# rdspring1/lightning-thunder

Measured on AMD Instinct MI355X. Metric: tokens/sec/GPU Llama-2-7B pretrain (LitGPT) + speedup vs eager at 1/2/4/8 MI355X, higher is better.
Workload: dtype bf16; 1 GPU; model=Llama-2-7b-hf, global_batch=1, micro_batch=1, seq_len=4096, parallelism=single, mode=thunder, optimizer=AdamW

## Files before the change

### lightning_thunder_amd/ops/csrc/gemm4.hip

```cpp
#include "common.h"

using namespace lta;

namespace {

typedef __bf16 bf16x8 __attribute__((ext_vector_type(8)));
typedef short s16x4 __attribute__((ext_vector_type(4)));
typedef float f32x4 __attribute__((ext_vector_type(4)));
typedef int i32x4 __attribute__((ext_vector_type(4)));
typedef __attribute__((address_space(3))) void lds_void;
typedef __attribute__((address_space(3))) s16x4 lds_s16x4;

constexpr int BM = 256, BN = 256, BK = 64, NTHR = 256;
constexpr int OP_BYTES = BM * BK * 2;
constexpr int STAGE = 2 * OP_BYTES;

enum Act : int { kNone = 0, kGeluTanh = 1, kGeluErf = 2, kSilu = 3, kRelu = 4 };

template <int ACT>
__device__ __forceinline__ float act_fn(float x) {
  if constexpr (ACT == kGeluTanh) {
    const float u = 0.7978845608028654f * (x + 0.044715f * x * x * x);
    return 0.5f * x * (1.f + tanhf(u));
  } else if constexpr (ACT == kGeluErf) {
    return 0.5f * x * (1.f + erff(x * 0.7071067811865476f));
  } else if constexpr (ACT == kSilu) {
    return x / (1.f + __expf(-x));
  } else if constexpr (ACT == kRelu) {
    return x > 0.f ? x : 0.f;
  } else {
    return x;
  }
}

__device__ __forceinline__ int xcd_tile(int orig, int nwg) {
  const int xcd = orig & 7, q = nwg >> 3, r = nwg & 7;
  return (xcd < r ? xcd * (q + 1) : r * (q + 1) + (xcd - r) * q) + (orig >> 3);
}

__device__ __forceinline__ int tr_swz(int k) { return ((k & 3) | (((k >> 3) & 1) << 2)) << 1; }

__device__ __forceinline__ i32x4 make_rsrc(const void* base, int bytes) {
  const uint64_t a = (uint64_t)(uintptr_t)base;
  return i32x4{(int)(uint32_t)a, (int)((uint32_t)(a >> 32) & 0xffffu), bytes, 0x00020000};
}

template <bool MN, bool DUAL = false, bool KEDGE = false>
struct Stager {
  i32x4 rsrc, rsrc2;
  const char* kbase;
  int kred, ldb2;
  int voff[8];
  int istride, kstride;
  __device__ __forceinline__ void init(const __hip_bfloat16* X, int ld, int r0, int K, int wave, int lane,
                                       const __hip_bfloat16* X2 = nullptr, int valid = BM) {
    if constexpr (DUAL) {
      rsrc = make_rsrc(X + (int64_t)r0 * ld, (BM / 2 - 1) * ld * 2 + K * 2);
      rsrc2 = make_rsrc(X2 + (int64_t)r0 * ld, (BM / 2 - 1) * ld * 2 + K * 2);
      const int r = lane >> 3, c = (lane & 7) ^ r;
      voff[0] = ((wave * 8 + r) * ld + c * 8) * 2;
      istride = 32 * ld * 2;
      kstride = BK * 2;
    } else if constexpr (!MN) {
      const __hip_bfloat16* base = X + (int64_t)r0 * ld;
      rsrc = make_rsrc(base, (BM - 1) * ld * 2 + K * 2);
      const int r = lane >> 3, c = (lane & 7) ^ r;
#pragma unroll
      for (int i = 0; i < 8; ++i) voff[i] = (min(32 * i + wave * 8 + r, valid - 1) * ld + c * 8) * 2;
      istride = 0;
      kstride = BK * 2;
    } else {
      const __hip_bfloat16* base = X + r0;
      rsrc = make_rsrc(base, (K - 1) * ld * 2 + BM * 2);
      const int half = lane >> 5, slot = lane & 31;
      const int kr = 2 * wave + half;
      const int c0 = slot ^ tr_swz(kr), cmax = (valid >> 3) - 1;
      if constexpr (KEDGE) {
#pragma unroll
        for (int i = 0; i < 8; ++i) voff[i] = ((8 * i + kr) * ld + min((i & 1) ? c0 ^ 8 : c0, cmax) * 8) * 2;
        kbase = reinterpret_cast<const char*>(base);
        kred = K;
        ldb2 = ld * 2;
      } else {
        voff[0] = (kr * ld + min(c0, cmax) * 8) * 2;
        voff[1] = (kr * ld + min(c0 ^ 8, cmax) * 8) * 2;
      }
      istride = 8 * ld * 2;
      kstride = BK * ld * 2;
    }
  }
  __device__ __forceinline__ void issue(int i, int kt, char* img, int wave) const {
    const uint32_t dst = (uint32_t)(uintptr_t)(__attribute__((address_space(3))) char*)(img + (i * 4 + wave) * 1024);
    if constexpr (KEDGE) {
      const int rows = max(0, min(BK, kred - kt * BK));
      const uint64_t a = (uint64_t)(uintptr_t)(kbase + (int64_t)kt * BK * ldb2);
      const i32x4 rk = i32x4{__builtin_amdgcn_readfirstlane((int)(uint32_t)a),
                             __builtin_amdgcn_readfirstlane((int)((uint32_t)(a >> 32) & 0xffffu)),
                             __builtin_amdgcn_readfirstlane(rows * ldb2), 0x00020000};
      asm volatile("s_mov_b32 m0, %0\n\ts_nop 0\n\tbuffer_load_dwordx4 %1, %2, 0 offen lds"
                   :
                   : "s"(dst), "v"(voff[i]), "s"(rk)
                   : "memory", "m0");
      return;
    }
    const bool second = DUAL && ((i >> 1) & 1);
    const int vo = DUAL ? voff[0] : (MN ? voff[i & 1] : voff[i]);
    const int so = DUAL ? (2 * (i >> 2) + (i & 1)) * istride + kt * kstride
                        : (MN ? i * istride + kt * kstride : kt * kstride);
    asm volatile("s_mov_b32 m0, %0\n\ts_nop 0\n\tbuffer_load_dwordx4 %1, %2, %3 offen lds"
                 :
                 : "s"(dst), "v"(vo), "s"(second ? rsrc2 : rsrc), "s"(so)
                 : "memory", "m0");
  }
};

template <bool MN>
__device__ __forceinline__ bf16x8 read_frag(const char* img, int rc, int kk, int fr, int fq) {
  if constexpr (!MN) {
    const int row = rc + fr;
    return *reinterpret_cast<const bf16x8*>(img + row * 128 + (((kk * 4 + fq) ^ (fr & 7)) << 4));
  } else {
    const int q = fr >> 2, p = fr & 3;
    const int k = kk * 32 + fq * 8 + q;
    const int c = (rc >> 3) + (p >> 1);
    const char* a0 = img + k * 512 + ((c ^ tr_swz(k)) << 4) + 8 * (p & 1);
    const char* a1 = img + (k + 4) * 512 + ((c ^ tr_swz(k + 4)) << 4) + 8 * (p & 1);
    const s16x4 lo = __builtin_amdgcn_ds_read_tr16_b64_v4i16((lds_s16x4*)(__attribute__((address_space(3))) char*)a0);
    const s16x4 hi = __builtin_amdgcn_ds_read_tr16_b64_v4i16((lds_s16x4*)(__attribute__((address_space(3))) char*)a1);
    union {
      struct {
        s16x4 a, b;
      } s;
      bf16x8 f;
    } u;
    u.s.a = lo;
    u.s.b = hi;
    return u.f;
  }
}

#define LTA_FENCE() __builtin_amdgcn_sched_barrier(0)

__device__ __forceinline__ void mfma16(f32x4& acc, const bf16x8& a, const bf16x8& b) {
  asm volatile("v_mfma_f32_16x16x32_bf16 %0, %1, %2, %0" : "+a"(acc) : "v"(a), "v"(b));
}

__device__ __forceinline__ float sigmoid_f(float x) { return 1.f / (1.f + __expf(-x)); }

__device__ __forceinline__ float bf16_round(float x) { return __bfloat162float(__float2bfloat16(x)); }

typedef float f32x2_t __attribute__((ext_vector_type(2)));
typedef __bf16 bf16x2_t __attribute__((ext_vector_type(2)));
__device__ __forceinline__ uint32_t pack_bf16x2(float lo, float hi) {
  return __builtin_bit_cast(uint32_t, __builtin_convertvector(f32x2_t{lo, hi}, bf16x2_t));
}

__device__ __forceinline__ uint4 swap_pair(uint32_t x0, uint32_t x1, uint32_t y0, uint32_t y1) {
  const auto s0 = __builtin_amdgcn_permlane16_swap(x0, y0, false, false);
  const auto s1 = __builtin_amdgcn_permlane16_swap(x1, y1, false, false);
  return make_uint4(s0[0], s1[0], s0[1], s1[1]);
}

struct EpiArgs {
  const __hip_bfloat16* B2;
  __hip_bfloat16* C2;
  __hip_bfloat16* C3;
  const __hip_bfloat16* R2;
  const float* cos_;
  const float* sin_;
  int T, nh, ng;
  const int* offs;
  int G;
  int64_t bstride, cstride;
  int tile_base, tile_count, ksplit;
  float* partial;
};

__device__ __forceinline__ void tile_coords(int wg, int nTm, int nTn, int& tm, int& tn) {
  constexpr int G = 8;
  const int per_group = G * nTn;
  const int group = wg / per_group;
  const int first_m = group * G;
  const int gm = min(nTm - first_m, G);
  const int in_group = wg % per_group;
  tm = first_m + in_group % gm;
  tn = in_group / gm;
}

template <int ACT, bool BIAS, bool RES, bool AT, bool BT, int VAR, int EPI = 0, int GRP = 0, int TAIL = 0>
__global__ __launch_bounds__(NTHR, 1) void gemm4_bf16_kernel(const __hip_bfloat16* __restrict__ A,
                                                            const __hip_bfloat16* __restrict__ B,
                                                            __hip_bfloat16* __restrict__ C,
                                                            const __hip_bfloat16* __restrict__ bias,
                                                            const __hip_bfloat16* __restrict__ R, int M, int N, int K,
                                                            int lda, int ldb, int ldc, int ldr, float alpha,
                                                            EpiArgs ep = {}) {
  const __hip_bfloat16* const B2 = ep.B2;
  __hip_bfloat16* const C2 = ep.C2;
  __hip_bfloat16* const C3 = ep.C3;
  const __hip_bfloat16* const R2 = ep.R2;
  static_assert(EPI != 1 || (!AT && !BT && !BIAS && !RES && ACT == 0), "gate-up: forward layout, no other epilogue");
  static_assert(EPI != 3 || (!AT && !BT && !BIAS && !RES && ACT == 0), "qkv rope: forward layout, no other epilogue");
  static_assert(EPI != 2 || (!AT && BT && !BIAS && !RES && ACT == 0), "swiglu backward: dgrad layout only");
  static_assert(GRP == 0 || (EPI == 0 && !BIAS && !RES && ACT == 0), "grouped: plain products");
  static_assert(GRP != 1 || !AT, "grouped rows: A row-major");
  static_assert(GRP != 2 || (AT && BT), "grouped reduction: A and B stored [rows][.]");
  constexpr bool SW = true;
  __shared__ __attribute__((aligned(1024))) char smem[2 * STAGE];

  const int tid = threadIdx.x, lane = tid & 63;
  const int wave = __builtin_amdgcn_readfirstlane(tid >> 6);
  const int wm = wave >> 1, wn = wave & 1;
  const int fr = lane & 15, fq = lane >> 4;

  const int nTm = (M + BM - 1) / BM, nTn = (N + BN - 1) / BN, nwg = nTm * nTn;
  const __hip_bfloat16* Ag = A;
  const __hip_bfloat16* Bg = B;
  __hip_bfloat16* Cg = C;
  int Mlim = M, Kr = K, m0, n0;
  [[maybe_unused]] int wg_lin = 0, kpart = 0;
  if constexpr (GRP == 0) {
    int wg;
    if constexpr (TAIL == 2) {
      const int t = __builtin_amdgcn_readfirstlane((int)blockIdx.x / ep.ksplit);
      kpart = __builtin_amdgcn_readfirstlane((int)blockIdx.x - t * ep.ksplit);
      wg = ep.tile_base + t;
    }
    else if constexpr (TAIL == 1)
      wg = ep.tile_base + xcd_tile((int)blockIdx.x, ep.tile_count);
    else
      wg = xcd_tile((int)blockIdx.x, nwg);
    wg_lin = wg;
    int tm, tn;
    tile_coords(wg, nTm, nTn, tm, tn);
    m0 = tm * BM;
    n0 = tn * BN;
    if constexpr (TAIL == 2) {
      const int P = K / (2 * BK), q = __builtin_amdgcn_readfirstlane(P / ep.ksplit), r = P - q * ep.ksplit;
      const int k0 = (kpart * q + min(kpart, r)) * (2 * BK);
      Kr = (q + (kpart < r ? 1 : 0)) * (2 * BK);
      Ag = A + (AT ? (int64_t)k0 * lda : (int64_t)k0);
      Bg = B + (BT ? (int64_t)k0 * ldb : (int64_t)k0);
    }
  } else if constexpr (GRP == 1) {
    const int bid = (int)blockIdx.x, tn = bid % nTn;
    int slot = bid / nTn, g = 0, start = 0, end = 0;
    bool found = false;
    for (; g < ep.G; ++g) {
      end = ep.offs[g];
      const int tiles = (end - start + BM - 1) / BM;
      if (slot < tiles) {
        found = true;
        break;
      }
      slot -= tiles;
      start = end;
    }
    if (!found) return;
    m0 = start + slot * BM;
    n0 = tn * BN;
    Mlim = end;
    Bg = B + (int64_t)g * ep.bstride;
  } else {
    const int g = (int)blockIdx.x / nwg, t = (int)blockIdx.x % nwg;
    const int start = g ? ep.offs[g - 1] : 0, end = ep.offs[g];
    m0 = (t / nTn) * BM;
    n0 = (t % nTn) * BN;
    Ag = A + (int64_t)start * lda;
    Bg = B + (int64_t)start * ldb;
    Cg = C + (int64_t)g * ep.cstride;
// ... 510 lines not shown
  ep.tile_base = 0;
  ep.tile_count = nwg - tail;
  hipLaunchKernelGGL((gemm4_bf16_kernel<kNone, false, false, AT, BT, 1, 0, 0, 1>), dim3(nwg - tail), dim3(NTHR), 0, s,
                     (const __hip_bfloat16*)A, (const __hip_bfloat16*)B, (__hip_bfloat16*)C, nullptr, nullptr, M, N, K,
                     lda, ldb, ldc, 0, alpha, ep);
  ep.tile_base = nwg - tail;
  ep.tile_count = tail;
  ep.ksplit = 2;
  ep.partial = (float*)ws;
  hipLaunchKernelGGL((gemm4_bf16_kernel<kNone, false, false, AT, BT, 1, 0, 0, 2>), dim3(2 * tail), dim3(NTHR), 0, s,
                     (const __hip_bfloat16*)A, (const __hip_bfloat16*)B, (__hip_bfloat16*)C, nullptr, nullptr, M, N, K,
                     lda, ldb, ldc, 0, 1.f, ep);
  hipLaunchKernelGGL(gemm4_tail_fixup, dim3((unsigned)((int64_t)tail * (BM * BN / 8) / 256)), dim3(256), 0, s,
                     (const float*)ws, (__hip_bfloat16*)C, 2, nwg - tail, tail, M, N, ldc, alpha);
  return (int)hipGetLastError();
}

template <bool AT, bool BT>
int launch4_splitk(const void* A, const void* B, void* C, const void* bias, int M, int N, int K, int lda, int ldb,
                   int ldc, float alpha, int ksplit, void* ws, int64_t ws_bytes, hipStream_t s) {
  const int nwg = ((M + BM - 1) / BM) * ((N + BN - 1) / BN);
  if (ksplit < 2 || ksplit > 64 || K % (2 * BK) || K / (2 * BK) < ksplit || !ws ||
      ws_bytes < (int64_t)ksplit * nwg * BM * BN * 4)
    return -2;
  EpiArgs ep{};
  ep.tile_base = 0;
  ep.tile_count = nwg;
  ep.ksplit = ksplit;
  ep.partial = (float*)ws;
  hipLaunchKernelGGL((gemm4_bf16_kernel<kNone, false, false, AT, BT, 1, 0, 0, 2>), dim3(ksplit * nwg), dim3(NTHR), 0,
                     s, (const __hip_bfloat16*)A, (const __hip_bfloat16*)B, (__hip_bfloat16*)C, nullptr, nullptr, M, N,
                     K, lda, ldb, ldc, 0, 1.f, ep);
  hipLaunchKernelGGL(gemm4_tail_fixup, dim3((unsigned)((int64_t)nwg * (BM * BN / 8) / 256)), dim3(256), 0, s,
                     (const float*)ws, (__hip_bfloat16*)C, ksplit, 0, nwg, M, N, ldc, alpha,
                     (const __hip_bfloat16*)bias);
  return (int)hipGetLastError();
}

template <int ACT, bool AT, bool BT, int VAR>
int launch4(const void* A, const void* B, void* C, const void* bias, const void* R, int M, int N, int K, int lda,
            int ldb, int ldc, int ldr, float alpha, hipStream_t s) {
  dim3 grid(((M + BM - 1) / BM) * ((N + BN - 1) / BN)), block(NTHR);
#define LTA_G4(BI, RE)                                                                                            \
  hipLaunchKernelGGL((gemm4_bf16_kernel<ACT, BI, RE, AT, BT, VAR>), grid, block, 0, s, (const __hip_bfloat16*)A,  \
                     (const __hip_bfloat16*)B, (__hip_bfloat16*)C, (const __hip_bfloat16*)bias,                  \
                     (const __hip_bfloat16*)R, M, N, K, lda, ldb, ldc, ldr, alpha)
  if (bias && R) { LTA_G4(true, true); }
  else if (bias) { LTA_G4(true, false); }
  else if (R) { LTA_G4(false, true); }
  else { LTA_G4(false, false); }
#undef LTA_G4
  return (int)hipGetLastError();
}

template <int VAR>
int dispatch_layout(const void* A, const void* B, void* C, const void* bias, const void* R, int M, int N, int K,
                    int lda, int ldb, int ldc, int ldr, float alpha, int act, int at, int bt, hipStream_t s) {
  if (!at && !bt) {
    switch (act) {
      case kNone: return launch4<kNone, false, false, VAR>(A, B, C, bias, R, M, N, K, lda, ldb, ldc, ldr, alpha, s);
      case kGeluTanh: return launch4<kGeluTanh, false, false, VAR>(A, B, C, bias, R, M, N, K, lda, ldb, ldc, ldr, alpha, s);
      case kGeluErf: return launch4<kGeluErf, false, false, VAR>(A, B, C, bias, R, M, N, K, lda, ldb, ldc, ldr, alpha, s);
      case kSilu: return launch4<kSilu, false, false, VAR>(A, B, C, bias, R, M, N, K, lda, ldb, ldc, ldr, alpha, s);
      case kRelu: return launch4<kRelu, false, false, VAR>(A, B, C, bias, R, M, N, K, lda, ldb, ldc, ldr, alpha, s);
      default: return -1;
    }
  }
  if (act != kNone || bias) return -1;
  if (!at && bt) return launch4<kNone, false, true, VAR>(A, B, C, nullptr, R, M, N, K, lda, ldb, ldc, ldr, alpha, s);
  if (at && !bt) return launch4<kNone, true, false, VAR>(A, B, C, nullptr, R, M, N, K, lda, ldb, ldc, ldr, alpha, s);
  return launch4<kNone, true, true, VAR>(A, B, C, nullptr, R, M, N, K, lda, ldb, ldc, ldr, alpha, s);
}

}

LTA_EXPORT int lta_gemm4_bf16(const void* A, const void* B, void* C, const void* bias, const void* R, int M, int N,
                              int K, int lda, int ldb, int ldc, int ldr, float alpha, int act, int at, int bt,
                              int variant, hipStream_t s) {
  if (N % 8 || K % (2 * BK) || M <= 0 || N <= 0 || K <= 0) return -2;
  if (at && M % 8) return -2;
  const int64_t ea = at ? (int64_t)K * lda : (int64_t)M * lda, eb = bt ? (int64_t)K * ldb : (int64_t)N * ldb;
  if (ea * 2 >= (1ll << 31) || eb * 2 >= (1ll << 31)) return -2;
  if (variant != 1) return -1;
  return dispatch_layout<1>(A, B, C, bias, R, M, N, K, lda, ldb, ldc, ldr, alpha, act, at, bt, s);
}

LTA_EXPORT int lta_gemm4_bf16_ws(const void* A, const void* B, void* C, const void* bias, const void* R, int M, int N,
                                 int K, int lda, int ldb, int ldc, int ldr, float alpha, int act, int at, int bt,
                                 int variant, void* ws, int64_t ws_bytes, hipStream_t s) {
  if (ws && variant == 1 && act == kNone && !bias && !R && N % 8 == 0 && M > 0 && N > 0 && K > 0 && !(at && M % 8)) {
    const int64_t ea = at ? (int64_t)K * lda : (int64_t)M * lda, eb = bt ? (int64_t)K * ldb : (int64_t)N * ldb;
    if (ea * 2 < (1ll << 31) && eb * 2 < (1ll << 31)) {
      int rc = -1;
      if (!at && !bt) rc = launch4_tail<false, false>(A, B, C, M, N, K, lda, ldb, ldc, alpha, ws, ws_bytes, s);
      else if (!at && bt) rc = launch4_tail<false, true>(A, B, C, M, N, K, lda, ldb, ldc, alpha, ws, ws_bytes, s);
      else if (at && !bt) rc = launch4_tail<true, false>(A, B, C, M, N, K, lda, ldb, ldc, alpha, ws, ws_bytes, s);
      else rc = launch4_tail<true, true>(A, B, C, M, N, K, lda, ldb, ldc, alpha, ws, ws_bytes, s);
      if (rc != -1) return rc;
    }
  }
  return lta_gemm4_bf16(A, B, C, bias, R, M, N, K, lda, ldb, ldc, ldr, alpha, act, at, bt, variant, s);
}

LTA_EXPORT int lta_gemm4_bf16_splitk(const void* A, const void* B, void* C, const void* bias, int M, int N, int K,
                                     int lda, int ldb, int ldc, float alpha, int at, int bt, int ksplit, void* ws,
                                     int64_t ws_bytes, hipStream_t s) {
  if (N % 8 || M <= 0 || N <= 0 || K <= 0 || (at && M % 8) || (bias && (at || bt))) return -2;
  const int64_t ea = at ? (int64_t)K * lda : (int64_t)M * lda, eb = bt ? (int64_t)K * ldb : (int64_t)N * ldb;
  if (ea * 2 >= (1ll << 31) || eb * 2 >= (1ll << 31)) return -2;
  if (!at && !bt) return launch4_splitk<false, false>(A, B, C, bias, M, N, K, lda, ldb, ldc, alpha, ksplit, ws, ws_bytes, s);
  if (!at && bt) return launch4_splitk<false, true>(A, B, C, bias, M, N, K, lda, ldb, ldc, alpha, ksplit, ws, ws_bytes, s);
  if (at && !bt) return launch4_splitk<true, false>(A, B, C, bias, M, N, K, lda, ldb, ldc, alpha, ksplit, ws, ws_bytes, s);
  return launch4_splitk<true, true>(A, B, C, bias, M, N, K, lda, ldb, ldc, alpha, ksplit, ws, ws_bytes, s);
}

LTA_EXPORT int lta_gemm4_grouped(int mode, const void* A, const void* B, void* C, const void* offs, int G, int M, int N,
                                 int K, int lda, int ldb, int ldc, int64_t bstride, int64_t cstride, int bt,
                                 hipStream_t s) {
  if (G <= 0 || M <= 0 || N <= 0 || N % 8 || !offs) return -2;
  EpiArgs ep{};
  ep.offs = (const int*)offs;
  ep.G = G;
  ep.bstride = bstride;
  ep.cstride = cstride;
  const int nTn = (N + BN - 1) / BN;
  if (mode == 1) {
    if (K % (2 * BK) || K <= 0) return -2;
    const dim3 grid(((M + BM - 1) / BM + G) * nTn);
    if (bt)
      hipLaunchKernelGGL((gemm4_bf16_kernel<kNone, false, false, false, true, 1, 0, 1>), grid, dim3(NTHR), 0, s,
                         (const __hip_bfloat16*)A, (const __hip_bfloat16*)B, (__hip_bfloat16*)C, nullptr, nullptr, M,
                         N, K, lda, ldb, ldc, 0, 1.f, ep);
    else
      hipLaunchKernelGGL((gemm4_bf16_kernel<kNone, false, false, false, false, 1, 0, 1>), grid, dim3(NTHR), 0, s,
                         (const __hip_bfloat16*)A, (const __hip_bfloat16*)B, (__hip_bfloat16*)C, nullptr, nullptr, M,
                         N, K, lda, ldb, ldc, 0, 1.f, ep);
    return (int)hipGetLastError();
  }
  if (mode == 2) {
    if (M % 8) return -2;
    const dim3 grid(G * ((M + BM - 1) / BM) * nTn);
    hipLaunchKernelGGL((gemm4_bf16_kernel<kNone, false, false, true, true, 1, 0, 2>), grid, dim3(NTHR), 0, s,
                       (const __hip_bfloat16*)A, (const __hip_bfloat16*)B, (__hip_bfloat16*)C, nullptr, nullptr, M, N,
                       K, lda, ldb, ldc, 0, 1.f, ep);
    return (int)hipGetLastError();
  }
  return -1;
}

LTA_EXPORT int lta_gemm4_swiglu(const void* A, const void* B, const void* B2, void* C, void* C2, void* C3,
                                const void* R, const void* R2, int M, int Nh, int K, int lda, int ldb, int ldc,
                                int mode, hipStream_t s) {
  if (K % (2 * BK) || M <= 0 || Nh <= 0 || K <= 0) return -2;
  if ((int64_t)M * lda * 2 >= (1ll << 31)) return -2;
  const dim3 block(NTHR);
  const int nTm = (M + BM - 1) / BM;
  if (mode == 1) {
    if (Nh % (BN / 2) || !B2 || !C3 || (int64_t)Nh * ldb * 2 >= (1ll << 31)) return -2;
    const int N = 2 * Nh;
    hipLaunchKernelGGL((gemm4_bf16_kernel<kNone, false, false, false, false, 1, 1>), dim3(nTm * (N / BN)), block,
                       0, s, (const __hip_bfloat16*)A, (const __hip_bfloat16*)B, (__hip_bfloat16*)C, nullptr, nullptr,
                       M, N, K, lda, ldb, ldc, 0, 1.f,
                       EpiArgs{(const __hip_bfloat16*)B2, (__hip_bfloat16*)C2, (__hip_bfloat16*)C3, nullptr, nullptr,
                               nullptr, 0, 0, 0});
    return (int)hipGetLastError();
  }
// ... 25 lines not shown
```

### lightning_thunder_amd/ops/gemm.py

```python
from __future__ import annotations

import os as _os
from typing import NamedTuple

import torch

import ctypes
import functools

from ._lib import require, stream_ptr, check, register_signature, dcode, c_int, c_void_p, c_float, c_int64

ACT = {None: 0, "none": 0, "gelu_tanh": 1, "gelu": 2, "gelu_erf": 2, "silu": 3, "relu": 4}
TILE_M, TILE_N, TILE_K = 256, 256, 64
GEMM4_MIN_M = 64

register_signature("lta_gemm_nt_bf16_v", [c_void_p, c_void_p, c_void_p, c_void_p, c_void_p, c_int, c_int, c_int, c_int,
                                          c_int, c_int, c_int, c_float, c_int, c_int, c_void_p])


def _gemm4_shape(M: int, N: int, K: int) -> bool:
    return M >= GEMM4_MIN_M and N % 8 == 0 and K % 128 == 0


def _gemm8_shape(M: int, N: int, K: int) -> bool:
    return M % TILE_M == 0 and N % TILE_N == 0 and K % TILE_K == 0


def _hand_gemm_shape(M: int, N: int, K: int) -> bool:
    return _gemm4_shape(M, N, K) or _gemm8_shape(M, N, K)


def _rowmajor_2d(t: torch.Tensor) -> bool:
    return t.dim() == 2 and t.stride(1) == 1 and t.stride(0) % 8 == 0 and t.data_ptr() % 16 == 0


def _plain_2d(t: torch.Tensor) -> bool:
    return t.dtype == torch.bfloat16 and t.is_cuda and _rowmajor_2d(t)


def _residual_ok(r, shape=None, rows16: bool = True) -> bool:
    if r is None:
        return True
    if r.dtype != torch.bfloat16 or (shape is not None and tuple(r.shape) != shape):
        return False
    return _rowmajor_2d(r) if rows16 else r.stride(1) == 1


def gemm_nt_supported(a: torch.Tensor, b: torch.Tensor, bias=None, residual=None) -> bool:
    if a.dtype != torch.bfloat16 or b.dtype != torch.bfloat16 or not a.is_cuda:
        return False
    if not _gemm8_shape(a.shape[0], b.shape[0], a.shape[1]):
        return False
    return nt_epilogue_ok(a, b, bias, residual)


def nt_epilogue_ok(a: torch.Tensor, b: torch.Tensor, bias=None, residual=None) -> bool:
    if not (_rowmajor_2d(a) and _rowmajor_2d(b)):
        return False
    M, K = a.shape
    N = b.shape[0]
    if b.shape[1] != K:
        return False
    if bias is not None and (bias.dtype != torch.bfloat16 or bias.numel() != N or not bias.is_contiguous()
                             or bias.data_ptr() % 16):
        return False
    return _residual_ok(residual, (M, N))


def gemm_nt(a: torch.Tensor, b: torch.Tensor, *, bias=None, residual=None, act=None, alpha: float = 1.0,
            out: torch.Tensor | None = None, variant: int | None = None) -> torch.Tensor:
    lib = require()
    M, K = a.shape
    N = b.shape[0]
    if variant is None:
        variant = int(_os.environ.get("LTA_GEMM_VARIANT", "0"))
    if out is None:
        out = torch.empty((M, N), dtype=torch.bfloat16, device=a.device)
    rc = lib.lta_gemm_nt_bf16_v(a.data_ptr(), b.data_ptr(), out.data_ptr(),
                                None if bias is None else bias.data_ptr(),
                                None if residual is None else residual.data_ptr(), M, N, K, a.stride(0), b.stride(0),
                                out.stride(0), 0 if residual is None else residual.stride(0), alpha, ACT[act], variant,
                                stream_ptr(a.device))
    check(rc, "lta_gemm_nt_bf16")
    return out


register_signature("lta_gemm4_bf16", [c_void_p, c_void_p, c_void_p, c_void_p, c_void_p, c_int, c_int, c_int, c_int,
                                      c_int, c_int, c_int, c_float, c_int, c_int, c_int, c_int, c_void_p])
register_signature("lta_gemm4_bf16_splitk", [c_void_p, c_void_p, c_void_p, c_void_p, c_int, c_int, c_int, c_int, c_int,
                                             c_int, c_float, c_int, c_int, c_int, c_void_p, c_int64, c_void_p])
register_signature("lta_gemm4_bf16_ws", [c_void_p, c_void_p, c_void_p, c_void_p, c_void_p, c_int, c_int, c_int, c_int,
                                         c_int, c_int, c_int, c_float, c_int, c_int, c_int, c_int, c_void_p, c_int64,
                                         c_void_p])

_TAIL_SPLIT = _os.environ.get("LTA_GEMM_TAIL_SPLIT", "1") != "0"


_CUS: dict = {}
_WS: dict = {}


def _device_cus(device) -> int:
    idx = device.index if device.index is not None else torch.cuda.current_device()
    if idx not in _CUS:
        _CUS[idx] = int(torch.cuda.get_device_properties(idx).multi_processor_count)
    return _CUS[idx]


def tail_tiles(M: int, N: int, K: int, cus: int) -> int:
    if not _TAIL_SPLIT or K % 256:
        return 0
    nwg = -(-M // 256) * -(-N // 256)
    tail = nwg % cus
    return 0 if nwg <= cus or 2 * tail > cus else tail


_SPLITK = _os.environ.get("LTA_GEMM_SPLITK", "1") != "0"
_KT_US, _FIXED_US, _PARTIAL_US, _LAUNCH_US = 1.3, 4.5, 2 * 262144 / 5e6, 3.0


@functools.lru_cache(maxsize=4096)
def splitk_factor(M: int, N: int, K: int, cus: int) -> int:
    if not _SPLITK or K % 128:
        return 0
    nwg = -(-M // 256) * -(-N // 256)
    if 2 * nwg > cus:
        return 0
    pairs = K // 128
    best, best_t = 0, 2 * pairs * _KT_US + _FIXED_US
    for s in range(2, min(64, cus // nwg, pairs) + 1):
        t = 2 * -(-pairs // s) * _KT_US + _FIXED_US + nwg * s * _PARTIAL_US + _LAUNCH_US
        if t < best_t:
            best, best_t = s, t
    return best


def _workspace(need: int, device):
    if torch.cuda.is_current_stream_capturing():
        return torch.empty(need, dtype=torch.float32, device=device)
    key = (device.index, torch.cuda.current_stream(device).cuda_stream)
    ws = _WS.get(key)
    if ws is None or ws.numel() < need:
        ws = torch.empty(need, dtype=torch.float32, device=device)
        _WS[key] = ws
    return ws


def gemm4_layout(a: torch.Tensor, b: torch.Tensor):
    if a.dtype != torch.bfloat16 or b.dtype != torch.bfloat16 or not a.is_cuda or a.dim() != 2 or b.dim() != 2:
        return None
    M, K = a.shape
    N = b.shape[1]
    if b.shape[0] != K or not _gemm4_shape(M, N, K) or N == 0 or K == 0:
        return None
    la, lb = _operand_layout(a, M, K), _operand_layout(b, K, N)
    if la is None or lb is None:
        return None
    at = 0 if la[0] == 1 else 1
    bt = 1 if lb[0] == 1 else 0
    if at and M % 8:
        return None
    if (K if at else M) * la[1] * 2 >= 2 ** 31 or (K if bt else N) * lb[1] * 2 >= 2 ** 31:
        return None
    return at, bt, la[1], lb[1]


def matmul4(a: torch.Tensor, b: torch.Tensor, *, bias=None, residual=None, act=None, alpha: float = 1.0,
            out: torch.Tensor | None = None, variant: int = 1) -> torch.Tensor:
    lay = gemm4_layout(a, b)
    if lay is None:
        raise ValueError(f"matmul4: unsupported operands {tuple(a.shape)}{a.stride()} @ {tuple(b.shape)}{b.stride()}")
    M, N = a.shape[0], b.shape[1]
    if bias is not None:
        assert bias.dtype == torch.bfloat16 and bias.numel() == N and bias.is_contiguous()
        bias = _aligned_bias(bias)
    return _run(_gemm4_launch(a, lay, bias, residual, act, variant, None, (M, N)), a, b, bias, residual, alpha, out)
# ... 580 lines not shown
```

Before: 24670 tokens/s.

## Add persistent GEMM kernel overlapping next-tile prefetch with epilogue stores

Adds a persistent-grid bf16 GEMM variant that loops over output tiles per workgroup, staging the next tile's first K-slices into LDS while the current tile's epilogue writes results. It is routed for plain (no bias/residual/activation) GEMMs whose tile count exceeds the CU count, for a table of layouts and K ranges. Shared device helpers move into a header. The aim is to hide launch and prologue/epilogue latency and wave-quantization tails, at the cost of extra code paths and a routing table that may pick it for shapes where it is not better.

```diff
diff --git a/lightning_thunder_amd/ops/csrc/gemm4.hip b/lightning_thunder_amd/ops/csrc/gemm4.hip
--- a/lightning_thunder_amd/ops/csrc/gemm4.hip
+++ b/lightning_thunder_amd/ops/csrc/gemm4.hip
@@ -1,19 +1,10 @@
 #include "common.h"
+#include "gemm4_device.h"
 
 using namespace lta;
+using namespace lta::gemm4dev;
 
 namespace {
-
-typedef __bf16 bf16x8 __attribute__((ext_vector_type(8)));
-typedef short s16x4 __attribute__((ext_vector_type(4)));
-typedef float f32x4 __attribute__((ext_vector_type(4)));
-typedef int i32x4 __attribute__((ext_vector_type(4)));
-typedef __attribute__((address_space(3))) void lds_void;
-typedef __attribute__((address_space(3))) s16x4 lds_s16x4;
-
-constexpr int BM = 256, BN = 256, BK = 64, NTHR = 256;
-constexpr int OP_BYTES = BM * BK * 2;
-constexpr int STAGE = 2 * OP_BYTES;
 
 enum Act : int { kNone = 0, kGeluTanh = 1, kGeluErf = 2, kSilu = 3, kRelu = 4 };
 
@@ -33,133 +24,11 @@
   }
 }
 
-__device__ __forceinline__ int xcd_tile(int orig, int nwg) {
-  const int xcd = orig & 7, q = nwg >> 3, r = nwg & 7;
-  return (xcd < r ? xcd * (q + 1) : r * (q + 1) + (xcd - r) * q) + (orig >> 3);
-}
-
-__device__ __forceinline__ int tr_swz(int k) { return ((k & 3) | (((k >> 3) & 1) << 2)) << 1; }
-
-__device__ __forceinline__ i32x4 make_rsrc(const void* base, int bytes) {
-  const uint64_t a = (uint64_t)(uintptr_t)base;
-  return i32x4{(int)(uint32_t)a, (int)((uint32_t)(a >> 32) & 0xffffu), bytes, 0x00020000};
-}
-
-template <bool MN, bool DUAL = false, bool KEDGE = false>
-struct Stager {
-  i32x4 rsrc, rsrc2;
-  const char* kbase;
-  int kred, ldb2;
-  int voff[8];
-  int istride, kstride;
-  __device__ __forceinline__ void init(const __hip_bfloat16* X, int ld, int r0, int K, int wave, int lane,
-                                       const __hip_bfloat16* X2 = nullptr, int valid = BM) {
-    if constexpr (DUAL) {
-      rsrc = make_rsrc(X + (int64_t)r0 * ld, (BM / 2 - 1) * ld * 2 + K * 2);
-      rsrc2 = make_rsrc(X2 + (int64_t)r0 * ld, (BM / 2 - 1) * ld * 2 + K * 2);
-      const int r = lane >> 3, c = (lane & 7) ^ r;
-      voff[0] = ((wave * 8 + r) * ld + c * 8) * 2;
-      istride = 32 * ld * 2;
-      kstride = BK * 2;
-    } else if constexpr (!MN) {
-      const __hip_bfloat16* base = X + (int64_t)r0 * ld;
-      rsrc = make_rsrc(base, (BM - 1) * ld * 2 + K * 2);
-      const int r = lane >> 3, c = (lane & 7) ^ r;
-#pragma unroll
-      for (int i = 0; i < 8; ++i) voff[i] = (min(32 * i + wave * 8 + r, valid - 1) * ld + c * 8) * 2;
-      istride = 0;
-      kstride = BK * 2;
-    } else {
-      const __hip_bfloat16* base = X + r0;
-      rsrc = make_rsrc(base, (K - 1) * ld * 2 + BM * 2);
-      const int half = lane >> 5, slot = lane & 31;
-      const int kr = 2 * wave + half;
-      const int c0 = slot ^ tr_swz(kr), cmax = (valid >> 3) - 1;
-      if constexpr (KEDGE) {
-#pragma unroll
-        for (int i = 0; i < 8; ++i) voff[i] = ((8 * i + kr) * ld + min((i & 1) ? c0 ^ 8 : c0, cmax) * 8) * 2;
-        kbase = reinterpret_cast<const char*>(base);
-        kred = K;
-        ldb2 = ld * 2;
-      } else {
-        voff[0] = (kr * ld + min(c0, cmax) * 8) * 2;
-        voff[1] = (kr * ld + min(c0 ^ 8, cmax) * 8) * 2;
-      }
-      istride = 8 * ld * 2;
-      kstride = BK * ld * 2;
-    }
-  }
-  __device__ __forceinline__ void issue(int i, int kt, char* img, int wave) const {
-    const uint32_t dst = (uint32_t)(uintptr_t)(__attribute__((address_space(3))) char*)(img + (i * 4 + wave) * 1024);
-    if constexpr (KEDGE) {
-      const int rows = max(0, min(BK, kred - kt * BK));
-      const uint64_t a = (uint64_t)(uintptr_t)(kbase + (int64_t)kt * BK * ldb2);
-      const i32x4 rk = i32x4{__builtin_amdgcn_readfirstlane((int)(uint32_t)a),
-                             __builtin_amdgcn_readfirstlane((int)((uint32_t)(a >> 32) & 0xffffu)),
-                             __builtin_amdgcn_readfirstlane(rows * ldb2), 0x00020000};
-      asm volatile("s_mov_b32 m0, %0\n\ts_nop 0\n\tbuffer_load_dwordx4 %1, %2, 0 offen lds"
-                   :
-                   : "s"(dst), "v"(voff[i]), "s"(rk)
-                   : "memory", "m0");
-      return;
-    }
-    const bool second = DUAL && ((i >> 1) & 1);
-    const int vo = DUAL ? voff[0] : (MN ? voff[i & 1] : voff[i]);
-    const int so = DUAL ? (2 * (i >> 2) + (i & 1)) * istride + kt * kstride
-                        : (MN ? i * istride + kt * kstride : kt * kstride);
-    asm volatile("s_mov_b32 m0, %0\n\ts_nop 0\n\tbuffer_load_dwordx4 %1, %2, %3 offen lds"
-                 :
-                 : "s"(dst), "v"(vo), "s"(second ? rsrc2 : rsrc), "s"(so)
-                 : "memory", "m0");
-  }
-};
-
-template <bool MN>
-__device__ __forceinline__ bf16x8 read_frag(const char* img, int rc, int kk, int fr, int fq) {
-  if constexpr (!MN) {
-    const int row = rc + fr;
-    return *reinterpret_cast<const bf16x8*>(img + row * 128 + (((kk * 4 + fq) ^ (fr & 7)) << 4));
-  } else {
-    const int q = fr >> 2, p = fr & 3;
-    const int k = kk * 32 + fq * 8 + q;
-    const int c = (rc >> 3) + (p >> 1);
-    const char* a0 = img + k * 512 + ((c ^ tr_swz(k)) << 4) + 8 * (p & 1);
-    const char* a1 = img + (k + 4) * 512 + ((c ^ tr_swz(k + 4)) << 4) + 8 * (p & 1);
-    const s16x4 lo = __builtin_amdgcn_ds_read_tr16_b64_v4i16((lds_s16x4*)(__attribute__((address_space(3))) char*)a0);
-    const s16x4 hi = __builtin_amdgcn_ds_read_tr16_b64_v4i16((lds_s16x4*)(__attribute__((address_space(3))) char*)a1);
-    union {
-      struct {
-        s16x4 a, b;
-      } s;
-      bf16x8 f;
-    } u;
-    u.s.a = lo;
-    u.s.b = hi;
-    return u.f;
-  }
-}
-
 #define LTA_FENCE() __builtin_amdgcn_sched_barrier(0)
 
-__device__ __forceinline__ void mfma16(f32x4& acc, const bf16x8& a, const bf16x8& b) {
-  asm volatile("v_mfma_f32_16x16x32_bf16 %0, %1, %2, %0" : "+a"(acc) : "v"(a), "v"(b));
-}
-
 __device__ __forceinline__ float sigmoid_f(float x) { return 1.f / (1.f + __expf(-x)); }
 
 __device__ __forceinline__ float bf16_round(float x) { return __bfloat162float(__float2bfloat16(x)); }
-
-typedef float f32x2_t __attribute__((ext_vector_type(2)));
-typedef __bf16 bf16x2_t __attribute__((ext_vector_type(2)));
-__device__ __forceinline__ uint32_t pack_bf16x2(float lo, float hi) {
-  return __builtin_bit_cast(uint32_t, __builtin_convertvector(f32x2_t{lo, hi}, bf16x2_t));
-}
-
-__device__ __forceinline__ uint4 swap_pair(uint32_t x0, uint32_t x1, uint32_t y0, uint32_t y1) {
-  const auto s0 = __builtin_amdgcn_permlane16_swap(x0, y0, false, false);
-  const auto s1 = __builtin_amdgcn_permlane16_swap(x1, y1, false, false);
-  return make_uint4(s0[0], s1[0], s0[1], s1[1]);
-}
 
 struct EpiArgs {
   const __hip_bfloat16* B2;
@@ -175,17 +44,6 @@
   int tile_base, tile_count, ksplit;
   float* partial;
 };
-
-__device__ __forceinline__ void tile_coords(int wg, int nTm, int nTn, int& tm, int& tn) {
-  constexpr int G = 8;
-  const int per_group = G * nTn;
-  const int group = wg / per_group;
-  const int first_m = group * G;
-  const int gm = min(nTm - first_m, G);
-  const int in_group = wg % per_group;
-  tm = first_m + in_group % gm;
-  tn = in_group / gm;
-}
 
 template <int ACT, bool BIAS, bool RES, bool AT, bool BT, int VAR, int EPI = 0, int GRP = 0, int TAIL = 0>
 __global__ __launch_bounds__(NTHR, 1) void gemm4_bf16_kernel(const __hip_bfloat16* __restrict__ A,
@@ -862,6 +720,8 @@
   const int64_t ea = at ? (int64_t)K * lda : (int64_t)M * lda, eb = bt ? (int64_t)K * ldb : (int64_t)N * ldb;
   if (ea * 2 >= (1ll << 31) || eb * 2 >= (1ll << 31)) return -2;
   if (variant != 1) return -1;
+  const int rp = lta_gemm4p_dispatch(A, B, C, bias, R, M, N, K, lda, ldb, ldc, alpha, act, at, bt, s);
+  if (rp != -1) return rp;
   return dispatch_layout<1>(A, B, C, bias, R, M, N, K, lda, ldb, ldc, ldr, alpha, act, at, bt, s);
 }
 
diff --git a/lightning_thunder_amd/ops/csrc/gemm4_device.h b/lightning_thunder_amd/ops/csrc/gemm4_device.h
--- /dev/null
+++ b/lightning_thunder_amd/ops/csrc/gemm4_device.h
@@ -0,0 +1,155 @@
+#pragma once
+#include "common.h"
+
+namespace lta {
+namespace gemm4dev {
+
+typedef __bf16 bf16x8 __attribute__((ext_vector_type(8)));
+typedef short s16x4 __attribute__((ext_vector_type(4)));
+typedef float f32x4 __attribute__((ext_vector_type(4)));
+typedef int i32x4 __attribute__((ext_vector_type(4)));
+typedef __attribute__((address_space(3))) void lds_void;
+typedef __attribute__((address_space(3))) s16x4 lds_s16x4;
+
+constexpr int BM = 256, BN = 256, BK = 64, NTHR = 256;
+constexpr int OP_BYTES = BM * BK * 2;
+constexpr int STAGE = 2 * OP_BYTES;
+
+__device__ __forceinline__ int xcd_tile(int orig, int nwg) {
+  const int xcd = orig & 7, q = nwg >> 3, r = nwg & 7;
+  return (xcd < r ? xcd * (q + 1) : r * (q + 1) + (xcd - r) * q) + (orig >> 3);
+}
+
+__device__ __forceinline__ int tr_swz(int k) { return ((k & 3) | (((k >> 3) & 1) << 2)) << 1; }
+
+__device__ __forceinline__ i32x4 make_rsrc(const void* base, int bytes) {
+  const uint64_t a = (uint64_t)(uintptr_t)base;
+  return i32x4{(int)(uint32_t)a, (int)((uint32_t)(a >> 32) & 0xffffu), bytes, 0x00020000};
+}
+
+template <bool MN, bool DUAL = false, bool KEDGE = false>
+struct Stager {
+  i32x4 rsrc, rsrc2;
+  const char* kbase;
+  int kred, ldb2;
+  int voff[8];
+  int istride, kstride;
+  __device__ __forceinline__ void init(const __hip_bfloat16* X, int ld, int r0, int K, int wave, int lane,
+                                       const __hip_bfloat16* X2 = nullptr, int valid = BM) {
+    if constexpr (DUAL) {
+      rsrc = make_rsrc(X + (int64_t)r0 * ld, (BM / 2 - 1) * ld * 2 + K * 2);
+      rsrc2 = make_rsrc(X2 + (int64_t)r0 * ld, (BM / 2 - 1) * ld * 2 + K * 2);
+      const int r = lane >> 3, c = (lane & 7) ^ r;
+      voff[0] = ((wave * 8 + r) * ld + c * 8) * 2;
+      istride = 32 * ld * 2;
+      kstride = BK * 2;
+    } else if constexpr (!MN) {
+      const __hip_bfloat16* base = X + (int64_t)r0 * ld;
+      rsrc = make_rsrc(base, (BM - 1) * ld * 2 + K * 2);
+      const int r = lane >> 3, c = (lane & 7) ^ r;
+#pragma unroll
+      for (int i = 0; i < 8; ++i) voff[i] = (min(32 * i + wave * 8 + r, valid - 1) * ld + c * 8) * 2;
+      istride = 0;
+      kstride = BK * 2;
+    } else {
+      const __hip_bfloat16* base = X + r0;
+      rsrc = make_rsrc(base, (K - 1) * ld * 2 + BM * 2);
+      const int half = lane >> 5, slot = lane & 31;
+      const int kr = 2 * wave + half;
+      const int c0 = slot ^ tr_swz(kr), cmax = (valid >> 3) - 1;
+      if constexpr (KEDGE) {
+#pragma unroll
+        for (int i = 0; i < 8; ++i) voff[i] = ((8 * i + kr) * ld + min((i & 1) ? c0 ^ 8 : c0, cmax) * 8) * 2;
+        kbase = reinterpret_cast<const char*>(base);
+        kred = K;
+        ldb2 = ld * 2;
+      } else {
+        voff[0] = (kr * ld + min(c0, cmax) * 8) * 2;
+        voff[1] = (kr * ld + min(c0 ^ 8, cmax) * 8) * 2;
+      }
+      istride = 8 * ld * 2;
+      kstride = BK * ld * 2;
+    }
+  }
+  __device__ __forceinline__ void issue(int i, int kt, char* img, int wave) const {
+    const uint32_t dst = (uint32_t)(uintptr_t)(__attribute__((address_space(3))) char*)(img + (i * 4 + wave) * 1024);
+    if constexpr (KEDGE) {
+      const int rows = max(0, min(BK, kred - kt * BK));
+      const uint64_t a = (uint64_t)(uintptr_t)(kbase + (int64_t)kt * BK * ldb2);
+      const i32x4 rk = i32x4{__builtin_amdgcn_readfirstlane((int)(uint32_t)a),
+                             __builtin_amdgcn_readfirstlane((int)((uint32_t)(a >> 32) & 0xffffu)),
+                             __builtin_amdgcn_readfirstlane(rows * ldb2), 0x00020000};
+      asm volatile("s_mov_b32 m0, %0\n\ts_nop 0\n\tbuffer_load_dwordx4 %1, %2, 0 offen lds"
+                   :
+                   : "s"(dst), "v"(voff[i]), "s"(rk)
+                   : "memory", "m0");
+      return;
+    }
+    const bool second = DUAL && ((i >> 1) & 1);
+    const int vo = DUAL ? voff[0] : (MN ? voff[i & 1] : voff[i]);
+    const int so = DUAL ? (2 * (i >> 2) + (i & 1)) * istride + kt * kstride
+                        : (MN ? i * istride + kt * kstride : kt * kstride);
+    asm volatile("s_mov_b32 m0, %0\n\ts_nop 0\n\tbuffer_load_dwordx4 %1, %2, %3 offen lds"
+                 :
+                 : "s"(dst), "v"(vo), "s"(second ? rsrc2 : rsrc), "s"(so)
+                 : "memory", "m0");
+  }
+};
+
+template <bool MN>
+__device__ __forceinline__ bf16x8 read_frag(const char* img, int rc, int kk, int fr, int fq) {
+  if constexpr (!MN) {
+    const int row = rc + fr;
+    return *reinterpret_cast<const bf16x8*>(img + row * 128 + (((kk * 4 + fq) ^ (fr & 7)) << 4));
+  } else {
+    const int q = fr >> 2, p = fr & 3;
+    const int k = kk * 32 + fq * 8 + q;
+    const int c = (rc >> 3) + (p >> 1);
+    const char* a0 = img + k * 512 + ((c ^ tr_swz(k)) << 4) + 8 * (p & 1);
+    const char* a1 = img + (k + 4) * 512 + ((c ^ tr_swz(k + 4)) << 4) + 8 * (p & 1);
+    const s16x4 lo = __builtin_amdgcn_ds_read_tr16_b64_v4i16((lds_s16x4*)(__attribute__((address_space(3))) char*)a0);
+    const s16x4 hi = __builtin_amdgcn_ds_read_tr16_b64_v4i16((lds_s16x4*)(__attribute__((address_space(3))) char*)a1);
+    union {
+      struct {
+        s16x4 a, b;
+      } s;
+      bf16x8 f;
+    } u;
+    u.s.a = lo;
+    u.s.b = hi;
+    return u.f;
+  }
+}
+
+__device__ __forceinline__ void mfma16(f32x4& acc, const bf16x8& a, const bf16x8& b) {
+  asm volatile("v_mfma_f32_16x16x32_bf16 %0, %1, %2, %0" : "+a"(acc) : "v"(a), "v"(b));
+}
+
+typedef float f32x2_t __attribute__((ext_vector_type(2)));
+typedef __bf16 bf16x2_t __attribute__((ext_vector_type(2)));
+__device__ __forceinline__ uint32_t pack_bf16x2(float lo, float hi) {
+  return __builtin_bit_cast(uint32_t, __builtin_convertvector(f32x2_t{lo, hi}, bf16x2_t));
+}
+
+__device__ __forceinline__ uint4 swap_pair(uint32_t x0, uint32_t x1, uint32_t y0, uint32_t y1) {
+  const auto s0 = __builtin_amdgcn_permlane16_swap(x0, y0, false, false);
+  const auto s1 = __builtin_amdgcn_permlane16_swap(x1, y1, false, false);
+  return make_uint4(s0[0], s1[0], s0[1], s1[1]);
+}
+
+__device__ __forceinline__ void tile_coords(int wg, int nTm, int nTn, int& tm, int& tn) {
+  constexpr int G = 8;
+  const int per_group = G * nTn;
+  const int group = wg / per_group;
+  const int first_m = group * G;
+  const int gm = min(nTm - first_m, G);
+  const int in_group = wg % per_group;
+  tm = first_m + in_group % gm;
+  tn = in_group / gm;
+}
+
+}
+}
+
+int lta_gemm4p_dispatch(const void* A, const void* B, void* C, const void* bias, const void* R, int M, int N, int K,
+                        int lda, int ldb, int ldc, float alpha, int act, int at, int bt, hipStream_t s);
diff --git a/lightning_thunder_amd/ops/csrc/gemm4p.hip b/lightning_thunder_amd/ops/csrc/gemm4p.hip
--- /dev/null
+++ b/lightning_thunder_amd/ops/csrc/gemm4p.hip
@@ -0,0 +1,274 @@
+#include "common.h"
+#include "gemm4_device.h"
+
+#include <cstdlib>
+
+using namespace lta;
+using namespace lta::gemm4dev;
+
+namespace {
+
+#define LTA_FENCE() __builtin_amdgcn_sched_barrier(0)
+
+__device__ __forceinline__ void mfma16_first(f32x4& acc, const bf16x8& a, const bf16x8& b) {
+  asm volatile("v_mfma_f32_16x16x32_bf16 %0, %1, %2, 0" : "=a"(acc) : "v"(a), "v"(b));
+}
+
+constexpr int NB2 = 8, NA = 16 - NB2;
+constexpr int EPI_STORES = 32;
+
+template <bool AT, bool BT>
+__global__ __launch_bounds__(NTHR, 1) void gemm4p_bf16_kernel(const __hip_bfloat16* __restrict__ A,
+                                                             const __hip_bfloat16* __restrict__ B,
+                                                             __hip_bfloat16* __restrict__ C, int M, int N, int K,
+                                                             int lda, int ldb, int ldc, float alpha) {
+  __shared__ __attribute__((aligned(1024))) char smem[2 * STAGE];
+
+  const int tid = threadIdx.x, lane = tid & 63;
+  const int wave = __builtin_amdgcn_readfirstlane(tid >> 6);
+  const int wm = wave >> 1, wn = wave & 1;
+  const int fr = lane & 15, fq = lane >> 4;
+
+  const int nTm = M / BM, nTn = N / BN, nwg = nTm * nTn, nk = K / BK;
+  const int step = (int)gridDim.x;
+
+  Stager<AT> sa;
+  Stager<BT> sb;
+  int m0 = 0, n0 = 0;
+  auto setup = [&](int lin) {
+    int tm, tn;
+    tile_coords(xcd_tile(lin, nwg), nTm, nTn, tm, tn);
+    m0 = __builtin_amdgcn_readfirstlane(tm * BM);
+    n0 = __builtin_amdgcn_readfirstlane(tn * BN);
+    int ln = lane, la = lda, lb = ldb;
+    asm volatile("" : "+v"(ln), "+s"(la), "+s"(lb));
+    sa.init(A, la, m0, K, wave, ln);
+    sb.init(B, lb, n0, K, wave, ln);
+  };
+  auto glds_w = [&](int j, int kt, char* stage, int w) {
+    if (j < 8)
+      sa.issue(j, kt, stage, w);
+    else
+      sb.issue(j - 8, kt, stage + OP_BYTES, w);
+  };
+  auto glds = [&](int j, int kt, char* stage) { glds_w(j, kt, stage, wave); };
+  auto stage_first = [&]() {
+    int w = wave;
+    asm volatile("" : "+s"(w));
+#pragma unroll
+    for (int j = 0; j < 16; ++j) glds_w(j, 0, smem, w);
+#pragma unroll
+    for (int j = 0; j < NB2; ++j) glds_w(j, 1, smem + STAGE, w);
+  };
+
+  f32x4 acc[8][8];
+  bf16x8 fa0[8], fb0[8], fa1[8], fb1[8];
+  auto mma = [](f32x4& c, const bf16x8& a, const bf16x8& b) { mfma16(c, b, a); };
+  auto mma_first = [](f32x4& c, const bf16x8& a, const bf16x8& b) { mfma16_first(c, b, a); };
+  auto read_one = [&](const char* stage, int kk, int r, bf16x8* fa, bf16x8* fb) {
+    if (r == 0)
+      fa[0] = read_frag<AT>(stage, wm * 128, kk, fr, fq);
+    else if (r <= 8)
+      fb[r - 1] = read_frag<BT>(stage + OP_BYTES, wn * 128 + (r - 1) * 16, kk, fr, fq);
+    else
+      fa[r - 8] = read_frag<AT>(stage, wm * 128 + (r - 8) * 16, kk, fr, fq);
+  };
+
+  auto body = [&](int t, auto cur_c, auto first_c) {
+    constexpr int CUR = decltype(cur_c)::value;
+    constexpr bool FIRST = decltype(first_c)::value;
+    char* const bc = smem + CUR * STAGE;
+    char* const bn = smem + (CUR ^ 1) * STAGE;
+    const int t1 = min(t + 1, nk - 1), t2 = min(t + 2, nk - 1);
+#pragma unroll
+    for (int i = 0; i < 64; ++i) {
+      if constexpr (FIRST)
+        mma_first(acc[i >> 3][i & 7], fa0[i >> 3], fb0[i & 7]);
+      else
+        mma(acc[i >> 3][i & 7], fa0[i >> 3], fb0[i & 7]);
+      if ((i & 3) == 0) read_one(bc, 1, i >> 2, fa1, fb1);
+      if (NA > 0 && (i & 3) == 2 && (i >> 2) < NA) glds(NB2 + (i >> 2), t1, bn);
+      LTA_FENCE();
+    }
+#pragma unroll
+    for (int i = 0; i < 32; ++i) {
+      mma(acc[i >> 3][i & 7], fa1[i >> 3], fb1[i & 7]);
+      LTA_FENCE();
+    }
+    asm volatile("s_waitcnt vmcnt(0) lgkmcnt(0)" ::: "memory");
+    __builtin_amdgcn_s_barrier();
+    LTA_FENCE();
+#pragma unroll
+    for (int i = 32; i < 64; ++i) {
+      mma(acc[i >> 3][i & 7], fa1[i >> 3], fb1[i & 7]);
+      const int s = i - 32;
+      if ((s & 1) == 0)
+        read_one(bn, 0, s >> 1, fa0, fb0);
+      else if ((s & 3) == 1 && (s >> 2) < NB2)
+        glds(s >> 2, t2, bc);
+      LTA_FENCE();
+    }
+  };
+
+  int lin = (int)blockIdx.x;
+  setup(lin);
+  stage_first();
+  asm volatile("s_waitcnt vmcnt(%0)" ::"n"(NB2) : "memory");
+  __builtin_amdgcn_s_barrier();
+
+  for (;;) {
+#pragma unroll
+    for (int r = 0; r < 16; ++r) read_one(smem, 0, r, fa0, fb0);
+
+    body(0, std::integral_constant<int, 0>{}, std::true_type{});
+    body(1, std::integral_constant<int, 1>{}, std::false_type{});
+    for (int t = 2; t < nk; t += 2) {
+      body(t, std::integral_constant<int, 0>{}, std::false_type{});
+      body(t + 1, std::integral_constant<int, 1>{}, std::false_type{});
+    }
+
+    asm volatile("s_waitcnt vmcnt(0) lgkmcnt(0)" ::: "memory");
+    __builtin_amdgcn_s_barrier();
+
+    const int cm0 = m0, cn0 = n0;
+    const int nxt = lin + step;
+    const bool more = nxt < nwg;
+    if (more) {
+      setup(nxt);
+      stage_first();
+    }
+
+#pragma unroll
+    for (int m = 0; m < 8; ++m)
+#pragma unroll
+      for (int n = 0; n < 8; ++n) asm volatile("" : "+a"(acc[m][n]));
+    asm volatile("s_nop 15\n\ts_nop 15" ::: "memory");
+    {
+      int ln = lane;
+      asm volatile("" : "+v"(ln));
+      const int er = ln & 15, eq = ln >> 4;
+      const int rsel = eq & 1, csel = eq >> 1;
+#pragma unroll
+      for (int m = 0; m < 8; ++m) {
+        const int64_t grow = cm0 + wm * 128 + m * 16 + er;
+#pragma unroll
+        for (int np = 0; np < 4; ++np) {
+          const int n = 2 * np;
+          float v[2][4];
+#pragma unroll
+          for (int h = 0; h < 2; ++h)
+#pragma unroll
+            for (int j = 0; j < 4; ++j) v[h][j] = acc[m][n + h][j] * alpha;
+          const uint4 val = swap_pair(pack_bf16x2(v[0][0], v[0][1]), pack_bf16x2(v[0][2], v[0][3]),
+                                      pack_bf16x2(v[1][0], v[1][1]), pack_bf16x2(v[1][2], v[1][3]));
+          const int gcol = cn0 + wn * 128 + (n + rsel) * 16 + csel * 8;
+          *reinterpret_cast<uint4*>(C + grow * ldc + gcol) = val;
+          __builtin_amdgcn_sched_barrier(0);
+        }
+      }
+    }
+    if (!more) break;
+
+    asm volatile("s_waitcnt vmcnt(%0)" ::"n"(EPI_STORES + NB2) : "memory");
+    __builtin_amdgcn_s_barrier();
+    lin = nxt;
+  }
+}
+
+#undef LTA_FENCE
+
+int device_cus() {
+  static int cached[64] = {};
+  int dev = 0, n = 0;
+  if (hipGetDevice(&dev) != hipSuccess) return 256;
+  if (dev >= 0 && dev < 64 && cached[dev] > 0) return cached[dev];
+  if (hipDeviceGetAttribute(&n, hipDeviceAttributeMultiprocessorCount, dev) != hipSuccess || n <= 0) return 256;
+  if (dev >= 0 && dev < 64) cached[dev] = n;
+  return n;
+}
+
+int g_gemm4_persist = [] {
+  const char* e = getenv("LTA_GEMM4_PERSIST");
+  return (e && e[0] == '0') ? 0 : 1;
+}();
+
+struct Route {
+  int at, bt, kmin, kmax, rounds;
+};
+constexpr Route kRoutes[] = {
+    {0, 0, 128, 1024, 0},
+    {0, 1, 128, 1024, 0},
+    {1, 0, 128, 1024, 0},
+    {1, 1, 128, 4096, 0},
+    {0, 0, 4096, 4096, 3},
+};
+
+bool shape_ok(int M, int N, int K) {
+  return M > 0 && N > 0 && K > 0 && M % BM == 0 && N % BN == 0 && K % (2 * BK) == 0;
+}
+
+bool in_table(int K, int at, int bt, int tiles, int grid) {
+  const int rounds = (tiles + grid - 1) / grid;
+  for (const Route& r : kRoutes)
+    if (r.at == (at ? 1 : 0) && r.bt == (bt ? 1 : 0) && K >= r.kmin && K <= r.kmax && (r.rounds == 0 || rounds <= r.rounds))
+      return true;
+  return false;
+}
+
+int persistent_grid(int tiles, int cus) {
+  const int c8 = cus >= 8 ? (cus & ~7) : max(cus, 1);
+  return min(tiles, c8);
+}
+
+bool operands_ok(int M, int N, int K, int lda, int ldb, int at, int bt) {
+  const int64_t ea = at ? (int64_t)K * lda : (int64_t)M * lda, eb = bt ? (int64_t)K * ldb : (int64_t)N * ldb;
+  return ea * 2 < (1ll << 31) && eb * 2 < (1ll << 31);
+}
+
+template <bool AT, bool BT>
+int launch4p(const void* A, const void* B, void* C, int M, int N, int K, int lda, int ldb, int ldc, float alpha,
+             int grid, hipStream_t s) {
+  hipLaunchKernelGGL((gemm4p_bf16_kernel<AT, BT>), dim3(grid), dim3(NTHR), 0, s, (const __hip_bfloat16*)A,
+                     (const __hip_bfloat16*)B, (__hip_bfloat16*)C, M, N, K, lda, ldb, ldc, alpha);
+  return (int)hipGetLastError();
+}
+
+int launch_layout(const void* A, const void* B, void* C, int M, int N, int K, int lda, int ldb, int ldc, float alpha,
+                  int at, int bt, int grid, hipStream_t s) {
+  if (!at && !bt) return launch4p<false, false>(A, B, C, M, N, K, lda, ldb, ldc, alpha, grid, s);
+  if (!at && bt) return launch4p<false, true>(A, B, C, M, N, K, lda, ldb, ldc, alpha, grid, s);
+  if (at && !bt) return launch4p<true, false>(A, B, C, M, N, K, lda, ldb, ldc, alpha, grid, s);
+  return launch4p<true, true>(A, B, C, M, N, K, lda, ldb, ldc, alpha, grid, s);
+}
+
+}
+
+LTA_EXPORT int lta_gemm4_set_persist(int on) {
+  const int old = g_gemm4_persist;
+  g_gemm4_persist = on ? 1 : 0;
+  return old;
+}
+
+LTA_EXPORT int lta_gemm4p_routed(int M, int N, int K, int at, int bt, int has_bias, int has_res, int act, int cus) {
+  if (!g_gemm4_persist || has_bias || has_res || act != 0 || !shape_ok(M, N, K)) return 0;
+  if (cus <= 0) cus = device_cus();
+  const int tiles = (M / BM) * (N / BN);
+  return tiles > cus && in_table(K, at, bt, tiles, persistent_grid(tiles, cus)) ? 1 : 0;
+}
+
+int lta_gemm4p_dispatch(const void* A, const void* B, void* C, const void* bias, const void* R, int M, int N, int K,
+                        int lda, int ldb, int ldc, float alpha, int act, int at, int bt, hipStream_t s) {
+  if (!g_gemm4_persist || bias || R || act != 0 || !shape_ok(M, N, K) || !operands_ok(M, N, K, lda, ldb, at, bt))
+    return -1;
+  const int cus = device_cus(), tiles = (M / BM) * (N / BN), grid = persistent_grid(tiles, cus);
+  if (tiles <= cus || !in_table(K, at, bt, tiles, grid)) return -1;
+  return launch_layout(A, B, C, M, N, K, lda, ldb, ldc, alpha, at, bt, grid, s);
+}
+
+LTA_EXPORT int lta_gemm4p_bf16(const void* A, const void* B, void* C, int M, int N, int K, int lda, int ldb, int ldc,
+                               float alpha, int at, int bt, int max_wgs, hipStream_t s) {
+  if (!shape_ok(M, N, K) || !operands_ok(M, N, K, lda, ldb, at, bt)) return -2;
+  const int tiles = (M / BM) * (N / BN);
+  const int grid = max_wgs > 0 ? min(tiles, max_wgs) : persistent_grid(tiles, device_cus());
+  return launch_layout(A, B, C, M, N, K, lda, ldb, ldc, alpha, at, bt, grid, s);
+}
diff --git a/lightning_thunder_amd/ops/gemm.py b/lightning_thunder_amd/ops/gemm.py
--- a/lightning_thunder_amd/ops/gemm.py
+++ b/lightning_thunder_amd/ops/gemm.py
@@ -92,6 +92,10 @@
 register_signature("lta_gemm4_bf16_ws", [c_void_p, c_void_p, c_void_p, c_void_p, c_void_p, c_int, c_int, c_int, c_int,
                                          c_int, c_int, c_int, c_float, c_int, c_int, c_int, c_int, c_void_p, c_int64,
                                          c_void_p])
+register_signature("lta_gemm4p_bf16", [c_void_p, c_void_p, c_void_p, c_int, c_int, c_int, c_int, c_int, c_int, c_float,
+                                       c_int, c_int, c_int, c_void_p])
+register_signature("lta_gemm4p_routed", [c_int, c_int, c_int, c_int, c_int, c_int, c_int, c_int, c_int])
+register_signature("lta_gemm4_set_persist", [c_int])
 
 _TAIL_SPLIT = _os.environ.get("LTA_GEMM_TAIL_SPLIT", "1") != "0"
 
```

New measurement: 24750 tokens/s (median of 6 runs). No clear change (+0.3%).
